# DiligentGraphics/DiligentFX

Hardware: AMD Instinct MI355X
Metric: Mpixels/s full PBR+postFX chain @4K; %HBM roofline; 1/2/4/8-GPU scaling (higher is better)
Workload: dtype f32; 1 GPU; full chain PBR+SSR+SSAO+composite+TAA+Bloom+ToneMap 3840x2160 per GPU (BASELINE configs[3]); width=3840, height_per_gpu=2160, storage=fp32 planes, taa=bicubic, ssao=GTAO full-res, ssr=full-res rays, tonemap=Uncharted2+sRGB, ibl=static maps: the shade's apron copy is made once (mifx_postfx_set_static_ibl), fusion_mask=31

## Files before the change

diligentfx_amd/csrc/taa.hip:

```cpp
#include "mifx_host.h"
#include "mifx_composite.h"

namespace mifx
{
mifx_status make_lutk(const mifx_image2d* im, LutK& k);

template <bool YCOCG> MIFX_D v3 rgb_to_ycocg(v3 c)
{
    if (!YCOCG) return c;
    const float co = c.x - c.z;
    const float t  = c.z + 0.5f * co;
    const float cg = c.y - t;
    const float yy = t + 0.5f * cg;
    return v3{yy, co, cg};
}
template <bool YCOCG> MIFX_D v3 ycocg_to_rgb(v3 c)
{
    if (!YCOCG) return c;
    const float t = c.x - 0.5f * c.z;
    const float g = c.z + t;
    const float b = t - 0.5f * c.y;
    const float r = b + c.y;
    return v3{r, g, b};
}
MIFX_D v3 hdr_to_sdr(v3 c) { return c * (mk3(1.0f) / (mk3(1.0f) + c)); }
MIFX_D v3 sdr_to_hdr(v3 c) { return c * (mk3(1.0f) / (mk3(1.0f) - c + mk3(5.960464478e-8f))); }

constexpr int kTaaBX = 32, kTaaBY = 8, kTaaTW = kTaaBX + 2, kTaaTH = kTaaBY + 2;
struct TaaCompositeIn
{
    Img   color, specIBL, ssao, normalTex, baseColor, material;
    LutK  lut;
    CamK  cam;
    float ssrScale, ssaoScale;
    int   outW, outH;
    SsrCleanupIn r7;
};
template <bool GAUSS, bool BICUBIC, bool YCOCG, bool COMPOSITE>
#ifndef MIFX_TAA_WAVES
#define MIFX_TAA_WAVES 5
#endif
__global__ __launch_bounds__(256) MIFX_WAVES(MIFX_TAA_WAVES) void taa_kernel(Img currColor, Img prevColor, Img motionTex, Img currDepth , Img prevDepth, Img out, CamK cur, CamK prev,
                                                  float stability, int reset, int skipRejection, TaaCompositeIn ci)
{
    __shared__ v4 tile[kTaaTH * kTaaTW];
    const int by0 = int(blockIdx.y) * kTaaBY + out.y0;
    const int x = blockIdx.x * kTaaBX + threadIdx.x;
    const int y = by0 + int(threadIdx.y);
    const int W = int(cur.vw), H = int(cur.vh);
    auto sample_curr = [&](int px, int py) {
        if (COMPOSITE)
        {
            v4 c;
            composite_pixel<MIFX_TONE_MAPPING_MODE_NONE, true>(c, px, py, ci.color, ci.specIBL, Img{}, ci.ssao, ci.normalTex, ci.baseColor, ci.material, ci.lut, ci.outW, ci.outH, ci.cam, ci.ssrScale,
                                                               ci.ssaoScale, ToneMapK{}, ci.r7);
            return max3(xyz(quantize_v4(c)), 0.0f);
        }
        return max3(xyz(ld<v4>(currColor, px, py)), 0.0f);
    };
    const bool inImage = x < out.w && y < row_end(out);
    v2    m;
    float cd;
    v3    ownColor = mk3(0.0f);
    float dtap[9] = {0.0f, 0.0f, 0.0f, 0.0f, 0.0f, 0.0f, 0.0f, 0.0f, 0.0f};
    {
        const int ox = blockIdx.x * kTaaBX - 1, oy = by0 - 1;
        if (COMPOSITE)
        {
            m  = inImage ? ld<cm_t>(motionTex, x, y) : v2{0.0f, 0.0f};
            cd = inImage ? ld<float>(currDepth, x, y) : 0.0f;
            auto fill = [&](int tx, int ty) {
                const v3 c = sample_curr(clampi(ox + tx, 0, W - 1), clampi(oy + ty, 0, H - 1));
                tile[ty * kTaaTW + tx] = mk4(rgb_to_ycocg<YCOCG>(hdr_to_sdr(c)), 0.0f);
                return c;
            };
            ownColor = fill(int(threadIdx.x) + 1, int(threadIdx.y) + 1);
            const int hh = int(threadIdx.y) * kTaaBX + int(threadIdx.x);
            if (hh < 2 * kTaaTW + 2 * kTaaBY)
            {
                const int tx = hh < kTaaTW ? hh : hh < 2 * kTaaTW ? hh - kTaaTW : hh < 2 * kTaaTW + kTaaBY ? 0 : kTaaTW - 1;
                const int ty = hh < kTaaTW ? 0 : hh < 2 * kTaaTW ? kTaaTH - 1 : hh < 2 * kTaaTW + kTaaBY ? 1 + hh - 2 * kTaaTW : 1 + hh - 2 * kTaaTW - kTaaBY;
                (void)fill(tx, ty);
            }
        }
        else
        {
            const int xc = min(x, out.w - 1), yc = min(y, row_end(out) - 1);
            m  = ld_once<cm_t>(motionTex, xc, yc);
            cd = ld_once<float>(currDepth, xc, yc);
            const int  i0 = int(threadIdx.y) * kTaaBX + int(threadIdx.x);
            const bool two = i0 + kTaaBX * kTaaBY < kTaaTW * kTaaTH;
            const int  i1 = two ? i0 + kTaaBX * kTaaBY : i0;
            v4 raw0 = ld<v4>(currColor, clampi(ox + i0 % kTaaTW, 0, W - 1), clampi(oy + i0 / kTaaTW, 0, H - 1));
            v4 raw1 = ld<v4>(currColor, clampi(ox + i1 % kTaaTW, 0, W - 1), clampi(oy + i1 / kTaaTW, 0, H - 1));
            keep_here(m);
            {
                const v2 mo{m.x * 0.5f, m.y * -0.5f};
                const v2 pp{(float(x) + 0.5f) - mo.x * cur.vw, (float(y) + 0.5f) - mo.y * cur.vh};
                const int pxi = int(pp.x), pyi = int(pp.y);
                for (int dy = -1; dy <= 1; ++dy)
                    for (int dx = -1; dx <= 1; ++dx) dtap[(dy + 1) * 3 + dx + 1] = ld_zero_f_nb(prevDepth, pxi + dx, pyi + dy);
            }
            keep_here(raw0);
            keep_here(raw1);
            tile[i0] = mk4(rgb_to_ycocg<YCOCG>(hdr_to_sdr(max3(xyz(raw0), 0.0f))), 0.0f);
            if (two) tile[i1] = mk4(rgb_to_ycocg<YCOCG>(hdr_to_sdr(max3(xyz(raw1), 0.0f))), 0.0f);
        }
#ifdef MIFX_TAA_LDS_BARRIER
        if (!COMPOSITE) asm volatile("s_waitcnt lgkmcnt(0)\n\ts_barrier" ::: "memory");
        else __syncthreads();
#else
        __syncthreads();
#endif
        if (!COMPOSITE)
            for (int i = 0; i < 9; ++i) keep_here(dtap[i]);
    }
    if (x >= out.w || y >= row_end(out)) return;
    auto tile_at = [&](int dx, int dy) { return xyz(tile[(int(threadIdx.y) + 1 + dy) * kTaaTW + int(threadIdx.x) + 1 + dx]); };
    const v2 pos{float(x) + 0.5f, float(y) + 0.5f};
    const v2 motion{m.x * 0.5f, m.y * -0.5f};
    const v2 prevPos{pos.x - motion.x * cur.vw, pos.y - motion.y * cur.vh};

    const bool inside = prevPos.x >= 0.0f && prevPos.y >= 0.0f && prevPos.x < cur.vw && prevPos.y < cur.vh;
    if (!inside || reset)
    {
        st<v4>(out, x, y, mk4(COMPOSITE ? ownColor : sample_curr(x, y), 0.5f));
        return;
    }
    const float aspect       = cur.vw * cur.ivh;
    const float motionFactor = saturate(1.0f - length(v2{motion.x * aspect, motion.y}) * 256.0f);

    bool similar = false;
    {
        const int   pxi = int(prevPos.x), pyi = int(prevPos.y);
        const float zc  = depth_to_camera_z(cd, cur.proj);
        constexpr float k = 0.105360515657826f;
        const float da = camera_z_to_depth(zc * (1.0f - k), prev.proj), db = camera_z_to_depth(fdiv(zc, 1.0f - k), prev.proj);
        const float dlo = fminf(da, db), dhi = fmaxf(da, db);
        for (int dy = -1; dy <= 1; ++dy)
            for (int dx = -1; dx <= 1; ++dx)
            {
                const float pd = COMPOSITE ? ld_zero_f_nb(prevDepth, pxi + dx, pyi + dy) : dtap[(dy + 1) * 3 + dx + 1];
                similar = similar || (pd > dlo && pd < dhi);
            }
    }
    const float depthFactor = similar ? 1.0f : 0.0f;
    v4 prevRGBA;
    if (BICUBIC)
    {
        const v2 texel{cur.ivw, cur.ivh};
        const v2 centre{floorf(prevPos.x - 0.5f) + 0.5f, floorf(prevPos.y - 0.5f) + 0.5f};
        const v2 f = prevPos - centre, f2 = f * f, f3 = f2 * f;
        const v2 w0 = -0.5f * f3 + f2 - 0.5f * f;
        const v2 w1 = 1.5f * f3 - 2.5f * f2 + 1.0f;
        const v2 w2 = -1.5f * f3 + 2.0f * f2 + 0.5f * f;
        const v2 w3 = 0.5f * f3 - 0.5f * f2;
        const v2 w12 = w1 + w2;
        const v2 tp0  = (centre - 1.0f) * texel;
        const v2 tp3  = (centre + 2.0f) * texel;
        const v2 tp12 = (centre + w2 / w12) * texel;
        const float p0 = w12.x * w0.y, p1 = w0.x * w12.y, p2 = w12.x * w12.y, p3 = w3.x * w12.y, p4 = w12.x * w3.y;
        v4 r = mk4(0.0f);
        r += sample_linear_clamp_v4(prevColor, tp12.x, tp0.y) * p0;
        r += sample_linear_clamp_v4(prevColor, tp0.x, tp12.y) * p1;
        r += sample_linear_clamp_v4(prevColor, tp12.x, tp12.y) * p2;
        r += sample_linear_clamp_v4(prevColor, tp3.x, tp12.y) * p3;
        r += sample_linear_clamp_v4(prevColor, tp12.x, tp3.y) * p4;
        prevRGBA = max4(r * fdiv(1.0f, p0 + p1 + p2 + p3 + p4), 0.0f);
    }
    else
    {
        prevRGBA = max4(sample_linear_clamp_v4(prevColor, prevPos.x * cur.ivw, prevPos.y * cur.ivh), 0.0f);
    }

    const v3 currY = tile_at(0, 0);
    const v3 prevY = rgb_to_ycocg<YCOCG>(hdr_to_sdr(xyz(prevRGBA)));
    auto corrected_alpha = [&](float a) { return fminf(stability, saturate(fdiv(1.0f, 2.0f - a))); };

    if (skipRejection)
    {
        const v3 o = sdr_to_hdr(ycocg_to_rgb<YCOCG>(lerp3(currY, prevY, prevRGBA.w)));
        st<v4>(out, x, y, mk4(o, corrected_alpha(prevRGBA.w)));
        return;
    }
    const float varianceGamma = lerpf(0.75f, 2.5f, motionFactor * motionFactor);

    float wsum = 0.0f;
    v3 m1 = mk3(0.0f), m2 = mk3(0.0f);
    for (int dx = -1; dx <= 1; ++dx)
        for (int dy = -1; dy <= 1; ++dy)
        {
            const v3    sdr = tile_at(dx, dy);
            const float w   = GAUSS ? expf(-3.0f * float(dx * dx + dy * dy) / ((1.0f + 1.0f) * (1.0f + 1.0f))) : 1.0f;
            m1 += sdr * w;
            m2 += sdr * sdr * w;
            wsum += w;
        }
    const v3 mean = m1 / wsum;
    const v3 var  = m2 / wsum - (mean * mean);
    const v3 sd   = sqrt3(max3(var, 0.0f));

    const float maxT = 10.0f;
    const v3 extents = varianceGamma * sd;
    const v3 dir     = currY - prevY;
    const v3 sgn{signf(dir.x), signf(dir.y), signf(dir.z)};
    const v3 isect   = ((mean - sgn * extents) - prevY) / dir;
    auto sel = [&](float i) { float ge = i >= 0.0f ? 1.0f : 0.0f; return (maxT + 1.0f) + ge * (i - (maxT + 1.0f)); };
    const v3 possible{sel(isect.x), sel(isect.y), sel(isect.z)};
    const float T = fminf(maxT, fminf(possible.x, fminf(possible.y, possible.z)));
    const float lt = T < maxT ? 1.0f : 0.0f;
    const v3 clamped = prevY + lt * ((prevY + dir * T) - prevY);

    const float alpha = prevRGBA.w * motionFactor * depthFactor;
    const v3 o = sdr_to_hdr(ycocg_to_rgb<YCOCG>(lerp3(currY, clamped, alpha)));
    st<v4>(out, x, y, mk4(o, corrected_alpha(alpha)));
}

mifx_status launch_taa(hipStream_t s, Img currColor, Img prevColor, Img motion, Img reprojDepth, Img prevDepth, Img out, const CamK& cur, const CamK& prev,
                       const mifx_taa_attribs& a, uint32_t flags, const TaaFusedComposite* fused)
{
    const dim3 block(kTaaBX, kTaaBY, 1), grid = grid2d(out, block);
    TaaCompositeIn ci{};
    if (fused)
    {
        const mifx_composite_attribs& ca = *fused->attribs;
        const uint32_t W = uint32_t(out.w), H = uint32_t(out.h);
        MIFX_CHECK(to_img_wh(ca.color, MIFX_FORMAT_F32X4, W, H, "color", ci.color));
        MIFX_CHECK(to_img_wh(ca.specular_ibl, MIFX_FORMAT_F32X4, W, H, "specular_ibl", ci.specIBL));
        MIFX_CHECK(to_img_wh(ca.ssao, MIFX_PLANE_AO, W, H, "ssao", ci.ssao));
        MIFX_CHECK(to_img_wh(ca.normal, MIFX_FORMAT_F32X4, W, H, "normal", ci.normalTex));
        MIFX_CHECK(to_img_wh(ca.base_color, MIFX_FORMAT_F32X4, W, H, "base_color", ci.baseColor));
        MIFX_CHECK(to_img_wh(ca.material, MIFX_FORMAT_F32X4, W, H, "material", ci.material));
        MIFX_REQUIRE(ca.camera != nullptr && fused->r7 != nullptr, "fused composite: camera and cleanup inputs must not be null");
        MIFX_REQUIRE(ca.tone_mapping == nullptr || ca.tone_mapping->iToneMappingMode == MIFX_TONE_MAPPING_MODE_NONE, "fused composite: the chain composites without a tone map while TAA is on");
        MIFX_CHECK(make_lutk(ca.brdf_lut, ci.lut));
        ci.cam = make_camk(*ca.camera);
        ci.ssrScale = ca.ssr_scale; ci.ssaoScale = ca.ssao_scale;
        ci.outW = out.w; ci.outH = out.h;
        ci.r7 = *fused->r7;
    }
#define MIFX_TAA_C(G, B, Y, C) hipLaunchKernelGGL((taa_kernel<G, B, Y, C>), grid, block, 0, s, currColor, prevColor, motion, reprojDepth, prevDepth, out, cur, prev, \
                                                  a.TemporalStabilityFactor, a.ResetAccumulation, a.SkipRejection, ci)
#define MIFX_TAA(G, B, Y) do { if (fused) MIFX_TAA_C(G, B, Y, true); else MIFX_TAA_C(G, B, Y, false); } while (0)
    switch (flags & 7u)
    {
        case 0: MIFX_TAA(false, false, false); break;
        case 1: MIFX_TAA(true, false, false); break;
        case 2: MIFX_TAA(false, true, false); break;
        case 3: MIFX_TAA(true, true, false); break;
        case 4: MIFX_TAA(false, false, true); break;
        case 5: MIFX_TAA(true, false, true); break;
        case 6: MIFX_TAA(false, true, true); break;
        default: MIFX_TAA(true, true, true); break;
    }
#undef MIFX_TAA
#undef MIFX_TAA_C
    MIFX_HIP_CHECK(hipGetLastError());
    return MIFX_OK;
}
}
```

Measured before the change: 5304 Mpixels/s.

## Fuse composite into TAA with rolling row-strip ring buffer to cut halo recompute

Adds a new fused composite+TAA kernel that walks vertical strips of rows with a 64-lane wave per row group and keeps composited rows in an LDS ring buffer. Each composited pixel is now computed roughly once instead of recomputing the 2D halo apron per 32x8 tile. It also gathers the previous-depth taps into registers ahead of the barrier. The old kernel is kept for the non-fused path. Trade-offs: a barrier per row group, serial iteration within each strip, lower parallelism per block, and two wasted edge lanes out of every 64.

```diff
diff --git a/diligentfx_amd/csrc/taa.hip b/diligentfx_amd/csrc/taa.hip
--- a/diligentfx_amd/csrc/taa.hip
+++ b/diligentfx_amd/csrc/taa.hip
@@ -1,5 +1,6 @@
 #include "mifx_host.h"
 #include "mifx_composite.h"
+#include <cstdlib>
 
 namespace mifx
 {
@@ -26,97 +27,10 @@
 MIFX_D v3 hdr_to_sdr(v3 c) { return c * (mk3(1.0f) / (mk3(1.0f) + c)); }
 MIFX_D v3 sdr_to_hdr(v3 c) { return c * (mk3(1.0f) / (mk3(1.0f) - c + mk3(5.960464478e-8f))); }
 
-constexpr int kTaaBX = 32, kTaaBY = 8, kTaaTW = kTaaBX + 2, kTaaTH = kTaaBY + 2;
-struct TaaCompositeIn
-{
-    Img   color, specIBL, ssao, normalTex, baseColor, material;
-    LutK  lut;
-    CamK  cam;
-    float ssrScale, ssaoScale;
-    int   outW, outH;
-    SsrCleanupIn r7;
-};
-template <bool GAUSS, bool BICUBIC, bool YCOCG, bool COMPOSITE>
-#ifndef MIFX_TAA_WAVES
-#define MIFX_TAA_WAVES 5
-#endif
-__global__ __launch_bounds__(256) MIFX_WAVES(MIFX_TAA_WAVES) void taa_kernel(Img currColor, Img prevColor, Img motionTex, Img currDepth , Img prevDepth, Img out, CamK cur, CamK prev,
-                                                  float stability, int reset, int skipRejection, TaaCompositeIn ci)
-{
-    __shared__ v4 tile[kTaaTH * kTaaTW];
-    const int by0 = int(blockIdx.y) * kTaaBY + out.y0;
-    const int x = blockIdx.x * kTaaBX + threadIdx.x;
-    const int y = by0 + int(threadIdx.y);
-    const int W = int(cur.vw), H = int(cur.vh);
-    auto sample_curr = [&](int px, int py) {
-        if (COMPOSITE)
-        {
-            v4 c;
-            composite_pixel<MIFX_TONE_MAPPING_MODE_NONE, true>(c, px, py, ci.color, ci.specIBL, Img{}, ci.ssao, ci.normalTex, ci.baseColor, ci.material, ci.lut, ci.outW, ci.outH, ci.cam, ci.ssrScale,
-                                                               ci.ssaoScale, ToneMapK{}, ci.r7);
-            return max3(xyz(quantize_v4(c)), 0.0f);
-        }
-        return max3(xyz(ld<v4>(currColor, px, py)), 0.0f);
-    };
-    const bool inImage = x < out.w && y < row_end(out);
-    v2    m;
-    float cd;
-    v3    ownColor = mk3(0.0f);
-    float dtap[9] = {0.0f, 0.0f, 0.0f, 0.0f, 0.0f, 0.0f, 0.0f, 0.0f, 0.0f};
-    {
-        const int ox = blockIdx.x * kTaaBX - 1, oy = by0 - 1;
-        if (COMPOSITE)
-        {
-            m  = inImage ? ld<cm_t>(motionTex, x, y) : v2{0.0f, 0.0f};
-            cd = inImage ? ld<float>(currDepth, x, y) : 0.0f;
-            auto fill = [&](int tx, int ty) {
-                const v3 c = sample_curr(clampi(ox + tx, 0, W - 1), clampi(oy + ty, 0, H - 1));
-                tile[ty * kTaaTW + tx] = mk4(rgb_to_ycocg<YCOCG>(hdr_to_sdr(c)), 0.0f);
-                return c;
-            };
-            ownColor = fill(int(threadIdx.x) + 1, int(threadIdx.y) + 1);
-            const int hh = int(threadIdx.y) * kTaaBX + int(threadIdx.x);
-            if (hh < 2 * kTaaTW + 2 * kTaaBY)
-            {
-                const int tx = hh < kTaaTW ? hh : hh < 2 * kTaaTW ? hh - kTaaTW : hh < 2 * kTaaTW + kTaaBY ? 0 : kTaaTW - 1;
-                const int ty = hh < kTaaTW ? 0 : hh < 2 * kTaaTW ? kTaaTH - 1 : hh < 2 * kTaaTW + kTaaBY ? 1 + hh - 2 * kTaaTW : 1 + hh - 2 * kTaaTW - kTaaBY;
-                (void)fill(tx, ty);
-            }
-        }
-        else
-        {
-            const int xc = min(x, out.w - 1), yc = min(y, row_end(out) - 1);
-            m  = ld_once<cm_t>(motionTex, xc, yc);
-            cd = ld_once<float>(currDepth, xc, yc);
-            const int  i0 = int(threadIdx.y) * kTaaBX + int(threadIdx.x);
-            const bool two = i0 + kTaaBX * kTaaBY < kTaaTW * kTaaTH;
-            const int  i1 = two ? i0 + kTaaBX * kTaaBY : i0;
-            v4 raw0 = ld<v4>(currColor, clampi(ox + i0 % kTaaTW, 0, W - 1), clampi(oy + i0 / kTaaTW, 0, H - 1));
-            v4 raw1 = ld<v4>(currColor, clampi(ox + i1 % kTaaTW, 0, W - 1), clampi(oy + i1 / kTaaTW, 0, H - 1));
-            keep_here(m);
-            {
-                const v2 mo{m.x * 0.5f, m.y * -0.5f};
-                const v2 pp{(float(x) + 0.5f) - mo.x * cur.vw, (float(y) + 0.5f) - mo.y * cur.vh};
-                const int pxi = int(pp.x), pyi = int(pp.y);
-                for (int dy = -1; dy <= 1; ++dy)
-                    for (int dx = -1; dx <= 1; ++dx) dtap[(dy + 1) * 3 + dx + 1] = ld_zero_f_nb(prevDepth, pxi + dx, pyi + dy);
-            }
-            keep_here(raw0);
-            keep_here(raw1);
-            tile[i0] = mk4(rgb_to_ycocg<YCOCG>(hdr_to_sdr(max3(xyz(raw0), 0.0f))), 0.0f);
-            if (two) tile[i1] = mk4(rgb_to_ycocg<YCOCG>(hdr_to_sdr(max3(xyz(raw1), 0.0f))), 0.0f);
-        }
-#ifdef MIFX_TAA_LDS_BARRIER
-        if (!COMPOSITE) asm volatile("s_waitcnt lgkmcnt(0)\n\ts_barrier" ::: "memory");
-        else __syncthreads();
-#else
-        __syncthreads();
-#endif
-        if (!COMPOSITE)
-            for (int i = 0; i < 9; ++i) keep_here(dtap[i]);
-    }
-    if (x >= out.w || y >= row_end(out)) return;
-    auto tile_at = [&](int dx, int dy) { return xyz(tile[(int(threadIdx.y) + 1 + dy) * kTaaTW + int(threadIdx.x) + 1 + dx]); };
+template <bool GAUSS, bool BICUBIC, bool YCOCG, class TileAt, class OwnColor>
+__device__ __forceinline__ void taa_resolve(int x, int y, v2 m, float cd, const float (&dtap)[9], TileAt tile_at, OwnColor own_color, const Img& prevColor, const Img& out,
+                                            const CamK& cur, const CamK& prev, float stability, int reset, int skipRejection)
+{
     const v2 pos{float(x) + 0.5f, float(y) + 0.5f};
     const v2 motion{m.x * 0.5f, m.y * -0.5f};
     const v2 prevPos{pos.x - motion.x * cur.vw, pos.y - motion.y * cur.vh};
@@ -124,7 +38,7 @@
     const bool inside = prevPos.x >= 0.0f && prevPos.y >= 0.0f && prevPos.x < cur.vw && prevPos.y < cur.vh;
     if (!inside || reset)
     {
-        st<v4>(out, x, y, mk4(COMPOSITE ? ownColor : sample_curr(x, y), 0.5f));
+        st<v4>(out, x, y, mk4(own_color(), 0.5f));
         return;
     }
     const float aspect       = cur.vw * cur.ivh;
@@ -140,7 +54,7 @@
         for (int dy = -1; dy <= 1; ++dy)
             for (int dx = -1; dx <= 1; ++dx)
             {
-                const float pd = COMPOSITE ? ld_zero_f_nb(prevDepth, pxi + dx, pyi + dy) : dtap[(dy + 1) * 3 + dx + 1];
+                const float pd = dtap[(dy + 1) * 3 + dx + 1];
                 similar = similar || (pd > dlo && pd < dhi);
             }
     }
@@ -216,6 +130,135 @@
     st<v4>(out, x, y, mk4(o, corrected_alpha(alpha)));
 }
 
+constexpr int kTaaBX = 32, kTaaBY = 8, kTaaTW = kTaaBX + 2, kTaaTH = kTaaBY + 2;
+template <bool GAUSS, bool BICUBIC, bool YCOCG>
+#ifndef MIFX_TAA_WAVES
+#define MIFX_TAA_WAVES 5
+#endif
+__global__ __launch_bounds__(256) MIFX_WAVES(MIFX_TAA_WAVES) void taa_kernel(Img currColor, Img prevColor, Img motionTex, Img currDepth , Img prevDepth, Img out, CamK cur, CamK prev,
+                                                  float stability, int reset, int skipRejection)
+{
+    __shared__ v4 tile[kTaaTH * kTaaTW];
+    const int by0 = int(blockIdx.y) * kTaaBY + out.y0;
+    const int x = blockIdx.x * kTaaBX + threadIdx.x;
+    const int y = by0 + int(threadIdx.y);
+    const int W = int(cur.vw), H = int(cur.vh);
+    auto sample_curr = [&](int px, int py) { return max3(xyz(ld<v4>(currColor, px, py)), 0.0f); };
+    v2    m;
+    float cd;
+    float dtap[9];
+    {
+        const int ox = blockIdx.x * kTaaBX - 1, oy = by0 - 1;
+        const int xc = min(x, out.w - 1), yc = min(y, row_end(out) - 1);
+        m  = ld_once<cm_t>(motionTex, xc, yc);
+        cd = ld_once<float>(currDepth, xc, yc);
+        const int  i0 = int(threadIdx.y) * kTaaBX + int(threadIdx.x);
+        const bool two = i0 + kTaaBX * kTaaBY < kTaaTW * kTaaTH;
+        const int  i1 = two ? i0 + kTaaBX * kTaaBY : i0;
+        v4 raw0 = ld<v4>(currColor, clampi(ox + i0 % kTaaTW, 0, W - 1), clampi(oy + i0 / kTaaTW, 0, H - 1));
+        v4 raw1 = ld<v4>(currColor, clampi(ox + i1 % kTaaTW, 0, W - 1), clampi(oy + i1 / kTaaTW, 0, H - 1));
+        keep_here(m);
+        {
+            const v2 mo{m.x * 0.5f, m.y * -0.5f};
+            const v2 pp{(float(x) + 0.5f) - mo.x * cur.vw, (float(y) + 0.5f) - mo.y * cur.vh};
+            const int pxi = int(pp.x), pyi = int(pp.y);
+            for (int dy = -1; dy <= 1; ++dy)
+                for (int dx = -1; dx <= 1; ++dx) dtap[(dy + 1) * 3 + dx + 1] = ld_zero_f_nb(prevDepth, pxi + dx, pyi + dy);
+        }
+        keep_here(raw0);
+        keep_here(raw1);
+        tile[i0] = mk4(rgb_to_ycocg<YCOCG>(hdr_to_sdr(max3(xyz(raw0), 0.0f))), 0.0f);
+        if (two) tile[i1] = mk4(rgb_to_ycocg<YCOCG>(hdr_to_sdr(max3(xyz(raw1), 0.0f))), 0.0f);
+#ifdef MIFX_TAA_LDS_BARRIER
+        asm volatile("s_waitcnt lgkmcnt(0)\n\ts_barrier" ::: "memory");
+#else
+        __syncthreads();
+#endif
+        for (int i = 0; i < 9; ++i) keep_here(dtap[i]);
+    }
+    if (x >= out.w || y >= row_end(out)) return;
+    auto tile_at = [&](int dx, int dy) { return xyz(tile[(int(threadIdx.y) + 1 + dy) * kTaaTW + int(threadIdx.x) + 1 + dx]); };
+    taa_resolve<GAUSS, BICUBIC, YCOCG>(x, y, m, cd, dtap, tile_at, [&] { return sample_curr(x, y); }, prevColor, out, cur, prev, stability, reset, skipRejection);
+}
+
+struct TaaCompositeIn
+{
+    Img   color, specIBL, ssao, normalTex, baseColor, material;
+    LutK  lut;
+    CamK  cam;
+    float ssrScale, ssaoScale;
+    int   outW, outH;
+    SsrCleanupIn r7;
+};
+constexpr int kTaaRsLanes = 64, kTaaRsOutW = kTaaRsLanes - 2, kTaaRsGroup = 4, kTaaRsSlots = 16;
+#ifndef MIFX_TAA_RS_ROWS
+#define MIFX_TAA_RS_ROWS 32
+#endif
+#ifndef MIFX_TAA_RS_WAVES
+#define MIFX_TAA_RS_WAVES 4
+#endif
+struct TaaRowsArgs
+{
+    Img   prevColor, motionTex, currDepth , prevDepth, out;
+    CamK  cur, prev;
+    float stability;
+    int   reset, skipRejection, rows;
+    TaaCompositeIn ci;
+};
+template <bool GAUSS, bool BICUBIC, bool YCOCG>
+__global__ __launch_bounds__(256) MIFX_WAVES(MIFX_TAA_RS_WAVES) void taa_composite_rows_kernel(TaaRowsArgs args)
+{
+    __shared__ v4 ring[kTaaRsSlots * kTaaRsLanes];
+    const int lane = int(threadIdx.x), w = int(threadIdx.y);
+    const int x0 = int(blockIdx.x) * kTaaRsOutW - 1 + lane;
+    const bool column = lane >= 1 && lane <= kTaaRsOutW && x0 < args.out.w;
+    const int ya = args.out.y0 + int(blockIdx.y) * args.rows;
+    const int n  = min(args.rows, row_end(args.out) - ya);
+    v3 own = mk3(0.0f);
+    for (int s = -1; kTaaRsGroup * s - 1 < n; ++s)
+    {
+        const TaaRowsArgs& a = args;
+        const TaaCompositeIn& ci = args.ci;
+        const Img& out = args.out;
+        int x = x0;
+        asm volatile("" : "+v"(x));
+        const int W = int(a.cur.vw), H = int(a.cur.vh);
+        const int xc = clampi(x, 0, W - 1);
+        auto composite_row = [&](int j) {
+            v4 c;
+            composite_pixel<MIFX_TONE_MAPPING_MODE_NONE, true>(c, xc, clampi(ya + j, 0, H - 1), ci.color, ci.specIBL, Img{}, ci.ssao, ci.normalTex, ci.baseColor, ci.material, ci.lut,
+                                                               ci.outW, ci.outH, ci.cam, ci.ssrScale, ci.ssaoScale, ToneMapK{}, ci.r7);
+            const v3 col = max3(xyz(quantize_v4(c)), 0.0f);
+            ring[((j + 1) & (kTaaRsSlots - 1)) * kTaaRsLanes + lane] = mk4(rgb_to_ycocg<YCOCG>(hdr_to_sdr(col)), 0.0f);
+            return col;
+        };
+        const int r = kTaaRsGroup * s + w - 1, y = ya + r;
+        const bool resolve = column && r >= 0 && r < n;
+        const v3 ownColor = own;
+        const int xo = clampi(x, 0, out.w - 1), yo = clampi(y, ya, ya + n - 1);
+        v2    m  = ld_once<cm_t>(a.motionTex, xo, yo);
+        float cd = ld_once<float>(a.currDepth, xo, yo);
+        if (r + kTaaRsGroup <= n) own = composite_row(r + kTaaRsGroup);
+        keep_here(m);
+        float dtap[9];
+        {
+            const v2 mo{m.x * 0.5f, m.y * -0.5f};
+            const v2 pp{(float(x) + 0.5f) - mo.x * a.cur.vw, (float(y) + 0.5f) - mo.y * a.cur.vh};
+            const int pxi = int(pp.x), pyi = int(pp.y);
+            for (int dy = -1; dy <= 1; ++dy)
+                for (int dx = -1; dx <= 1; ++dx) dtap[(dy + 1) * 3 + dx + 1] = ld_zero_f_nb(a.prevDepth, pxi + dx, pyi + dy);
+        }
+        asm volatile("s_waitcnt lgkmcnt(0)\n\ts_barrier" ::: "memory");
+        for (int i = 0; i < 9; ++i) keep_here(dtap[i]);
+        if (resolve)
+        {
+            auto tile_at = [&](int dx, int dy) { return xyz(ring[((r + 1 + dy) & (kTaaRsSlots - 1)) * kTaaRsLanes + lane + dx]); };
+            taa_resolve<GAUSS, BICUBIC, YCOCG>(x, y, m, cd, dtap, tile_at, [&] { return ownColor; }, a.prevColor, out, a.cur, a.prev, a.stability, a.reset,
+                                               a.skipRejection);
+        }
+    }
+}
+
 mifx_status launch_taa(hipStream_t s, Img currColor, Img prevColor, Img motion, Img reprojDepth, Img prevDepth, Img out, const CamK& cur, const CamK& prev,
                        const mifx_taa_attribs& a, uint32_t flags, const TaaFusedComposite* fused)
 {
@@ -239,9 +282,12 @@
         ci.outW = out.w; ci.outH = out.h;
         ci.r7 = *fused->r7;
     }
-#define MIFX_TAA_C(G, B, Y, C) hipLaunchKernelGGL((taa_kernel<G, B, Y, C>), grid, block, 0, s, currColor, prevColor, motion, reprojDepth, prevDepth, out, cur, prev, \
-                                                  a.TemporalStabilityFactor, a.ResetAccumulation, a.SkipRejection, ci)
-#define MIFX_TAA(G, B, Y) do { if (fused) MIFX_TAA_C(G, B, Y, true); else MIFX_TAA_C(G, B, Y, false); } while (0)
+    static const int stripRows = [] { const char* e = std::getenv("MIFX_TAA_RS_ROWS"); const int v = e ? std::atoi(e) : 0; return v > 0 ? v : MIFX_TAA_RS_ROWS; }();
+    const dim3 rsBlock(kTaaRsLanes, kTaaRsGroup, 1), rsGrid(unsigned(out.w + kTaaRsOutW - 1) / kTaaRsOutW, unsigned(window_rows(out) + stripRows - 1) / unsigned(stripRows), 1);
+    const TaaRowsArgs rs{prevColor, motion, reprojDepth, prevDepth, out, cur, prev, a.TemporalStabilityFactor, a.ResetAccumulation, a.SkipRejection, stripRows, ci};
+#define MIFX_TAA(G, B, Y) do { if (fused) hipLaunchKernelGGL((taa_composite_rows_kernel<G, B, Y>), rsGrid, rsBlock, 0, s, rs); \
+                               else hipLaunchKernelGGL((taa_kernel<G, B, Y>), grid, block, 0, s, currColor, prevColor, motion, reprojDepth, prevDepth, out, cur, prev, \
+                                                       a.TemporalStabilityFactor, a.ResetAccumulation, a.SkipRejection); } while (0)
     switch (flags & 7u)
     {
         case 0: MIFX_TAA(false, false, false); break;
@@ -254,7 +300,6 @@
         default: MIFX_TAA(true, true, true); break;
     }
 #undef MIFX_TAA
-#undef MIFX_TAA_C
     MIFX_HIP_CHECK(hipGetLastError());
     return MIFX_OK;
 }
```

Result: no change. 5296 Mpixels/s (median of 2 runs) (-0.1%).
